# yinghansun/pympc-quadruped

Hardware: AMD Instinct MI355X
Metric: QP solves/sec (whole node), horizon=10 GRF QP, at 1/2/4/8 MI355X (higher is better)
Workload: dtype f64; 1 GPU; config2: batch 1024/GPU, horizon 10, gaits trot10, robots a1; batch_per_gpu=1024, horizon=10, global_batch=1024, parallelism=robot-sharded x1

## Files before the change

pympc-quadruped_amd/csrc/mpcqp.hip:

```cpp

#include <hip/hip_runtime.h>

#include <math.h>
#include <stdint.h>

#include <cmath>
#include <string.h>

#include <new>
#include <string>
#include <type_traits>
#include <utility>
#include <vector>

#include "mpcqp.h"

namespace {

constexpr int NX = 13;
constexpr int NU = 12;
constexpr int LANES = 64;
constexpr int kMaxN = MPCQP_MAX_HORIZON;
constexpr int kDenseN = 20;
static_assert(kMaxN >= kDenseN && 4 * kMaxN <= 2 * LANES, "stance lists cover 4 N <= 128 entries");
// ... 225 lines not shown
      "s_nop 1\n\t"
      "v_min_f32_dpp %0, %0, %0 row_bcast:31 row_mask:0xc bank_mask:0xf"
      : "+v"(v));
  return __builtin_bit_cast(float, __builtin_amdgcn_readlane(__builtin_bit_cast(int, v), 63));
}
__device__ __forceinline__ int wave_argmin_d(double v, double& vmin_out) {
  const float f = (float)v;
  const float fm = wave_min_f32(f);
  const unsigned long long cand = __ballot(f == fm);
  int l;
  if (__popcll(cand) == 1) {
    l = uni(__builtin_ctzll(cand));
    vmin_out = readlane_d(v, l);
  } else if (fm == INFINITY && __ballot(v < INFINITY) == 0ull) {
    l = 0;
    vmin_out = INFINITY;
  } else {
    const double vv = (f == fm) ? v : INFINITY;
    const double m = wave_min(vv);
    l = uni(__builtin_ctzll(__ballot(vv == m)));
    vmin_out = m;
  }
  return l;
}

__device__ __forceinline__ int wave_argmin_f32(double v, double& vmin_out) {
  const float f = (float)v;
  const float fm = wave_min_f32(f);
  const int l = uni(__builtin_ctzll(__ballot(f == fm)));
  vmin_out = readlane_d(v, l);
  return l;
}

#include "mpcqp_form.h"
#include "mpcqp_combo_asm.h"
#include "mpcqp_solve.h"
#include "mpcqp_ipm.h"
#include "mpcqp_plan.h"
#include "mpcqp_swing.h"
#include "mpcqp_kinematics.h"
#include "mpcqp_estimator.h"
#include "mpcqp_attitude.h"
static_assert(MPCQP_KIN_STRIDE == KIN_STRIDE, "geometry record: include/mpcqp.h and mpcqp_kin_leg.h agree");

__device__ __forceinline__ int xcd_robot(int bid, int B) {
  const int x = bid & 7, i = bid >> 3, q = B >> 3, r = B & 7;
  return x * q + (x < r ? x : r) + i;
}

constexpr int kOrderMax = 8192;
constexpr int kOrderSeg = 1024;
constexpr int kOrderMin = 64;
constexpr int kOrderBuckets = 256;

__device__ __forceinline__ float order_key(const float* __restrict__ x0g, const float* __restrict__ xrefg, int N,
                                           int r) {
  const float ex = x0g[(size_t)r * NX + 9] - xrefg[(size_t)r * N * NX + 9];
  const float ey = x0g[(size_t)r * NX + 10] - xrefg[(size_t)r * N * NX + 10];
  const float k = ex * ex + ey * ey;
  return k >= 0.0f && k <= 3.0e38f ? k : 0.0f;
}

__global__ __launch_bounds__(1024) void mpcqp_order_kernel(int B, int N, const float* __restrict__ x0g,
                                                           const float* __restrict__ xrefg, int* __restrict__ perm,
                                                           int mode) {
  __shared__ int hist[kOrderBuckets], cursor[kOrderBuckets];
// ... 48 lines not shown
    }
    if (lane == LANES - 1) wsum[tid >> 6] = x;
    hist[tid] = x - v;
  }
  __syncthreads();
  if (tid < kOrderBuckets) {
    int off = 0;
    for (int w = 0; w < (tid >> 6); ++w) off += wsum[w];
    hist[tid] += off;
  }
  __syncthreads();
#pragma unroll
  for (int t = 0; t < KPT; ++t) {
    const int j = tid + 1024 * t;
    if (j < len) {
      const int pos = hist[bk[t]] + atomicAdd(&cursor[bk[t]], 1);
      perm[start + stride * pos] = start + stride * j;
    }
  }
}

constexpr int kCap64 = 64;
constexpr int kIpmPerCU = 4;
template <int NM, bool FULL, bool MG>
constexpr bool ipm_within_slots() {
  return sizeof(IpmSharedT<NM, FULL, MG>) > 160 * 1024 / (kIpmPerCU + 1);
}
static_assert(ipm_within_slots<16, false, true>() && ipm_within_slots<16, true, true>() &&
                  ipm_within_slots<16, false, false>() && ipm_within_slots<16, true, false>() &&
                  ipm_within_slots<kDenseN, false, false>() && ipm_within_slots<kDenseN, true, false>() &&
                  ipm_within_slots<kMaxN, false, false>() && ipm_within_slots<kMaxN, true, false>(),
              "an interior-point layout fits more workgroups on a CU than kIpmPerCU slots");

template <bool FULL>
__global__ __launch_bounds__(Cfg<64>::NT) __attribute__((amdgpu_waves_per_eu(2, Cfg<64>::NW))) void mpcqp_kernel_64(
    KParams P, int B, const float* __restrict__ x0g, const float* __restrict__ xrefg,
    const float* __restrict__ contactg, const float* __restrict__ feetg, const float* __restrict__ robotg,
    float* __restrict__ u0g, float* __restrict__ Ug, int* __restrict__ statusg, int* __restrict__ itersg,
    int* __restrict__ queue, int* __restrict__ queue_big, int* __restrict__ queue_ipm, const int* __restrict__ perm) {
  if ((int)blockIdx.x >= B) return;
  int b = xcd_robot(blockIdx.x, B);
  if (perm) b = uni(perm[b]);
  __shared__ SharedT<64> sm;
  solve_robot<64, FULL>(P, b, sm, x0g, xrefg, contactg, feetg, robotg, u0g, Ug, statusg, itersg, queue, queue_big,
                  queue_ipm);
}

template <bool FULL>
__global__ __launch_bounds__(Cfg<96>::NT) __attribute__((amdgpu_waves_per_eu((Cfg<96>::NW + 3) / 4, (Cfg<96>::NW + 3) / 4))) void mpcqp_kernel_96(
    KParams P, const float* __restrict__ x0g, const float* __restrict__ xrefg,
    const float* __restrict__ contactg, const float* __restrict__ feetg, const float* __restrict__ robotg,
    float* __restrict__ u0g, float* __restrict__ Ug, int* __restrict__ statusg, int* __restrict__ itersg,
    int* __restrict__ queue, int* __restrict__ qout, int* __restrict__ q_ipm, int direct_B,
    const int* __restrict__ perm) {
  __shared__ SharedT<96> sm;
  const int tid = threadIdx.x;
  const int k = blockIdx.x;
  if (direct_B > 0) {
    if (k < direct_B)
      solve_robot<96, FULL>(P, perm ? uni(perm[k]) : k, sm, x0g, xrefg, contactg, feetg, robotg, u0g, Ug, statusg,
                            itersg, qout, nullptr, q_ipm);
    return;
  }
  const int cnt = uni(__hip_atomic_load(&queue[0], __ATOMIC_RELAXED, __HIP_MEMORY_SCOPE_AGENT));
  if (k < cnt) {
    const int b = uni(queue[4 + k]);
    solve_robot<96, FULL>(P, b, sm, x0g, xrefg, contactg, feetg, robotg, u0g, Ug, statusg, itersg, qout, nullptr, q_ipm);
    if (tid == 0 && atomicAdd(&queue[2], 1) == cnt - 1) {
      atomicExch(&queue[0], 0);
      atomicExch(&queue[2], 0);
    }
  }
}

template <bool FULL>
__global__ __launch_bounds__(Cfg<128>::NT) void mpcqp_kernel_128(
    KParams P, const float* __restrict__ x0g, const float* __restrict__ xrefg,
    const float* __restrict__ contactg, const float* __restrict__ feetg, const float* __restrict__ robotg,
// ... 64 lines not shown
}

struct QueueSet {
  hipStream_t stream;
  int cap;
  int* buf;
  unsigned long long used;
  hipStream_t side;
  hipEvent_t ev_fork, ev_join;
  hipEvent_t ev_done;
};

static void release_set(QueueSet& q) {
  if (q.buf) (void)hipFree(q.buf);
  if (q.ev_fork) (void)hipEventDestroy(q.ev_fork);
  if (q.ev_join) (void)hipEventDestroy(q.ev_join);
  if (q.ev_done) (void)hipEventDestroy(q.ev_done);
  q.ev_done = nullptr;
  if (q.side) (void)hipStreamDestroy(q.side);
  q.buf = nullptr;
  q.ev_fork = q.ev_join = nullptr;
  q.side = nullptr;
}

struct mpcqp_ctx {
  mpcqp_params params;
  int device;
  int stance_hint;
  int stance_min;
  int order;
  int ncu;
  std::vector<QueueSet> queues;
  unsigned long long use_clock;
  double* sscratch;
  int sslots;
  double* wdev;
  bool xr;
  double q_full[13 * 13];
  double r_full[12 * 12];
  std::vector<double*> retired;
  unsigned char* warm;
  int warm_cap;
  double dt_control;
  double gravity;
  double max_pos_error;
  double swing_height;
  double touchdown_z;
  double vel_gain;
  double kp_swing[9];
  double kd_swing[9];
  EstParams est;
  AttParams att;
  std::string err;
};

static int set_err(mpcqp_ctx* ctx, int code, const std::string& msg) {
  if (ctx) ctx->err = msg;
  return code;
}

struct DeviceScope {
  int prev = -1;
  bool ok = false;
  explicit DeviceScope(int dev) {
    if (hipGetDevice(&prev) != hipSuccess) prev = -1;
    ok = hipSetDevice(dev) == hipSuccess;
// ... 102 lines not shown
  if (hipGetDeviceCount(&ndev) != hipSuccess || device < 0 || device >= ndev) return MPCQP_ERR_HIP;
  mpcqp_ctx* ctx = new (std::nothrow) mpcqp_ctx();
  if (!ctx) return MPCQP_ERR_ALLOC;
  ctx->params = *p;
  ctx->device = device;
  ctx->stance_hint = 0;
  ctx->stance_min = 0;
  ctx->order = 1;
  ctx->ncu = 0;
  ctx->use_clock = 0;
  ctx->sscratch = nullptr;
  ctx->sslots = 0;
  ctx->wdev = nullptr;
  ctx->xr = false;
  ctx->warm = nullptr;
  ctx->warm_cap = 0;
  for (int i = 0; i < 13 * 13; ++i) ctx->q_full[i] = (i % 14 == 0) ? p->q_diag[i / 14] : 0.0;
  for (int i = 0; i < 12 * 12; ++i) ctx->r_full[i] = (i % 13 == 0) ? p->r_diag[i / 13] : 0.0;
  ctx->dt_control = 0.001;
  ctx->gravity = 9.81;
  ctx->swing_height = 0.1;
  ctx->touchdown_z = -0.0255;
  ctx->vel_gain = 0.03;
  for (int i = 0; i < 9; ++i) {
    ctx->kp_swing[i] = i % 4 == 0 ? 700.0 : 0.0;
    ctx->kd_swing[i] = i % 4 == 0 ? 20.0 : 0.0;
  }
  ctx->max_pos_error = 0.1;
  ctx->est = EstParams{0, 0.001, 9.81, 0.001, 0.0098, 0.002, 0.001, 0.1, 0.001, 100.0, 100.0, 0.0};
  ctx->att = AttParams{0.001, 9.81, 0.1, 0.0, 0.2, 0.0};
  hipDeviceProp_t prop;
  if (hipGetDeviceProperties(&prop, device) == hipSuccess) ctx->ncu = prop.multiProcessorCount;
  if (ctx->ncu <= 0) ctx->ncu = 256;
  *out = ctx;
  return MPCQP_OK;
}

int mpcqp_set_warm_start(mpcqp_ctx* ctx, void* memory, int32_t capacity) {
  if (!ctx) return MPCQP_ERR_ARG;
  if (capacity < 0 || (capacity > 0 && !memory))
    return set_err(ctx, MPCQP_ERR_ARG, "warm start: capacity < 0, or no memory for capacity > 0");
  ctx->warm = capacity > 0 ? static_cast<unsigned char*>(memory) : nullptr;
  ctx->warm_cap = capacity > 0 ? capacity : 0;
  return MPCQP_OK;
}

int mpcqp_set_order(mpcqp_ctx* ctx, int32_t mode) {
  if (!ctx) return MPCQP_ERR_ARG;
  if (mode != 0 && mode != 1) return set_err(ctx, MPCQP_ERR_ARG, "order: mode must be 0 or 1");
  ctx->order = mode;
  return MPCQP_OK;
}

int mpcqp_set_stance_hint(mpcqp_ctx* ctx, int32_t max_stance) {
  return mpcqp_set_stance_range(ctx, 0, max_stance);
}

int mpcqp_set_stance_range(mpcqp_ctx* ctx, int32_t min_stance, int32_t max_stance) {
  if (!ctx) return MPCQP_ERR_ARG;
  if (min_stance < 0 || max_stance < 0 || (max_stance > 0 && min_stance > max_stance))
    return set_err(ctx, MPCQP_ERR_ARG, "stance range: min > max or negative");
  if (min_stance > 4 * ctx->params.horizon)
    return set_err(ctx, MPCQP_ERR_ARG, "stance range: min_stance > 4 * horizon");
  ctx->stance_min = min_stance;
  ctx->stance_hint = max_stance;
  return MPCQP_OK;
// ... 71 lines not shown
                       ctx->sscratch, sbits, ctx->sslots / 32);
    ipm_done = true;
    return hipGetLastError();
  };
  auto fork_ipm = [&]() -> int {
    if (!fork || ipm_done) return MPCQP_OK;
    if (hipEventRecord(qs->ev_fork, st) != hipSuccess || hipStreamWaitEvent(qs->side, qs->ev_fork, 0) != hipSuccess)
      return set_err(ctx, MPCQP_ERR_HIP, "interior-point fork failed");
    const hipError_t le = launch_ipm(qs->side);
    if (le != hipSuccess) return set_err(ctx, MPCQP_ERR_HIP, std::string("launch (ipm): ") + hipGetErrorString(le));
    if (hipEventRecord(qs->ev_join, qs->side) != hipSuccess) return set_err(ctx, MPCQP_ERR_HIP, "join record failed");
    return MPCQP_OK;
  };
  const size_t qstride = 4 + (size_t)cap;
  int* q1 = large ? q : nullptr;
  int* perm = use_order ? q + 3 * qstride : nullptr;
  int* q2 = huge ? q + qstride : nullptr;
  int* q3 = giant ? q + 2 * qstride : nullptr;
  hipError_t e = hipSuccess;
  int fe = MPCQP_OK;
  auto failed = [&](int code) -> int {
    if (fork && ipm_done) (void)hipStreamWaitEvent(st, qs->ev_join, 0);
    if (qs) (void)hipEventRecord(qs->ev_done, st);
    return code;
  };
  if (use_order) {
    const int segs = first == 0 ? 8 : (int)((batch + kOrderSeg - 1) / kOrderSeg);
    hipLaunchKernelGGL(mpcqp_order_kernel, dim3(segs), dim3(1024), 0, st, (int)batch, kp.N, x0, xref, perm,
                       first == 0 ? 0 : 1);
    e = hipGetLastError();
    if (e != hipSuccess) return failed(set_err(ctx, MPCQP_ERR_HIP, std::string("launch (order): ") + hipGetErrorString(e)));
  }
  if (first == 0) {
    hipLaunchKernelGGL(full ? mpcqp_kernel_64<true> : mpcqp_kernel_64<false>, dim3(batch), dim3(Cfg<64>::NT),
                       kDiagLds, st, kp, (int)batch, x0, xref, contact,
                       feet, robot, u0, U, (int*)status, (int*)iters, q1, q2, q3, perm);
    e = hipGetLastError();
    if (e != hipSuccess) return failed(set_err(ctx, MPCQP_ERR_HIP, std::string("launch: ") + hipGetErrorString(e)));
    if ((fe = fork_ipm()) != MPCQP_OK) return failed(fe);
  }
  if (large && first <= 1) {
    hipLaunchKernelGGL(full ? mpcqp_kernel_96<true> : mpcqp_kernel_96<false>, dim3(batch), dim3(Cfg<96>::NT), 0, st, kp, x0, xref, contact, feet, robot,
                       u0, U, (int*)status, (int*)iters, q1, q2, q3, first == 1 ? (int)batch : 0,
                       first == 1 ? perm : nullptr);
    e = hipGetLastError();
    if (e != hipSuccess) return failed(set_err(ctx, MPCQP_ERR_HIP, std::string("launch (96): ") + hipGetErrorString(e)));
    if ((fe = fork_ipm()) != MPCQP_OK) return failed(fe);
  }
  if (huge && first <= 2) {
    hipLaunchKernelGGL(full ? mpcqp_kernel_128<true> : mpcqp_kernel_128<false>, dim3(batch), dim3(Cfg<128>::NT), 0, st, kp, x0, xref, contact, feet, robot,
                       u0, U, (int*)status, (int*)iters, q2, q3, first == 2 ? (int)batch : 0,
                       first == 2 ? perm : nullptr);
    e = hipGetLastError();
    if (e != hipSuccess) return failed(set_err(ctx, MPCQP_ERR_HIP, std::string("launch (128): ") + hipGetErrorString(e)));
    if ((fe = fork_ipm()) != MPCQP_OK) return failed(fe);
  }
  if (giant && !ipm_done) {
    e = launch_ipm(st);
    if (e != hipSuccess) return failed(set_err(ctx, MPCQP_ERR_HIP, std::string("launch (ipm): ") + hipGetErrorString(e)));
  } else if (fork && hipStreamWaitEvent(st, qs->ev_join, 0) != hipSuccess) {
    return failed(set_err(ctx, MPCQP_ERR_HIP, "interior-point join failed"));
  }
  if (qs && hipEventRecord(qs->ev_done, st) != hipSuccess) return set_err(ctx, MPCQP_ERR_HIP, "queue event record failed");
  return MPCQP_OK;
}

int mpcqp_set_weights(mpcqp_ctx* ctx, const double* Q, const double* R) {
  if (!ctx) return MPCQP_ERR_ARG;
  double q[NX * NX], r[NU * NU];
// ... 305 lines not shown
  ctx->att = AttParams{dt, gravity, kappa_ref, bias_gain, trust_window, touch_threshold};
  return MPCQP_OK;
}

int mpcqp_attitude(mpcqp_ctx* ctx, int32_t batch, int32_t flags, const float* gyro, const float* accel,
                   const int32_t* tick, int32_t iterations_between_mpc, const int32_t* gait, const float* touch,
                   double* att_state, float* quat, float* gyro_out, float* trust, int32_t* status, void* stream) {
  if (!ctx) return MPCQP_ERR_ARG;
  if (flags != 0) return set_err(ctx, MPCQP_ERR_ARG, "unknown attitude flags");
  if (batch <= 0) return set_err(ctx, MPCQP_ERR_ARG, "attitude: batch <= 0");
  if (!gyro || !accel || !att_state) return set_err(ctx, MPCQP_ERR_ARG, "null attitude input/state pointer");
  if ((uintptr_t)att_state & 15) return set_err(ctx, MPCQP_ERR_ARG, "att_state is not 16-byte aligned");
  if (gait && !tick) return set_err(ctx, MPCQP_ERR_ARG, "attitude: gait given without tick");
  if (trust && !gait && !touch)
    return set_err(ctx, MPCQP_ERR_ARG, "attitude: trust wanted with neither gait and tick nor touch");
  if (gait && iterations_between_mpc < 1) return set_err(ctx, MPCQP_ERR_ARG, "attitude: iterations_between_mpc < 1");
  static_assert(ATT_STRIDE == MPCQP_ATT_STRIDE, "record stride");
  static_assert(ATT_STATUS_OK == MPCQP_STATUS_OK && ATT_STATUS_NONFINITE == MPCQP_STATUS_NONFINITE, "status words");
  DeviceScope dev(ctx->device);
  if (!dev.ok) return set_err(ctx, MPCQP_ERR_HIP, "hipSetDevice failed");
  hipLaunchKernelGGL(mpcqp_attitude_kernel, dim3((batch + kAttThreads - 1) / kAttThreads), dim3(kAttThreads), 0,
                     (hipStream_t)stream, ctx->att, (int)batch, (int)iterations_between_mpc, gyro, accel, tick, gait,
                     touch, att_state, quat, gyro_out, trust, status);
  const hipError_t e = hipGetLastError();
  if (e != hipSuccess) return set_err(ctx, MPCQP_ERR_HIP, std::string("attitude launch: ") + hipGetErrorString(e));
  return MPCQP_OK;
}

int mpcqp_destroy(mpcqp_ctx* ctx) {
  if (ctx) {
    DeviceScope dev(ctx->device);
    for (auto& q : ctx->queues) release_set(q);
    if (ctx->sscratch) (void)hipFree(ctx->sscratch);
    if (ctx->wdev) (void)hipFree(ctx->wdev);
    for (double* o : ctx->retired) (void)hipFree(o);
  }
  delete ctx;
  return MPCQP_OK;
}

const char* mpcqp_last_error(const mpcqp_ctx* ctx) { return ctx ? ctx->err.c_str() : "null context"; }

}
```

pympc-quadruped_amd/csrc/mpcqp_form.h:

```cpp

template <int NM>
struct alignas(16) FormT {
  static constexpr int IN_XREF = IN_CONTACT + 4 * NM, IN_END = IN_XREF + NX * NM;
  float in[IN_END];
  double K[3][NU];
  double G[3][NU];
  double E0[NM][16];
  double E1[NM][8];
  double ii[9];
  double rz[2];
  double minv;
  double q[16];
  double qf[NX * NX];
  double es[2][NM][NX];
  double X[2][NX][NU];
  double QX[2][NX][NU];
};
using Form = FormT<kDenseN>;

struct alignas(16) FormY {
  d2 Y[NU * NU];
  double rd2[NU];
  double Yf[3][NU * NU];
  double rf2[NU * NU];
// ... 180 lines not shown
    double a = 0.0;
#pragma unroll
    for (int j = 0; j < NX; ++j) a = fma(f.qf[i * NX + j], f.X[w][j][c], a);
    f.QX[w][i][c] = a;
  }
  for (int e = tid; e < N * NX; e += NT) {
    const int t = e / NX, sc = e % NX;
    double a0 = 0.0, a1 = 0.0;
#pragma unroll
    for (int j = 0; j < NX; ++j) {
      a0 = fma(f.qf[sc * NX + j], f.es[0][t][j], a0);
      a1 = fma(f.qf[sc * NX + j], f.es[1][t][j], a1);
    }
    f.E0[t][sc] = a0;
    if (sc < 6) f.E1[t][sc] = a1;
  }
  fsync<NT>();
  for (int e = tid; e < 3 * NU * NU; e += NT) {
    const int w = e / (NU * NU), c1 = (e / NU) % NU, c2 = e % NU;
    const int xa = w == 2 ? 1 : 0, qb = w == 0 ? 0 : 1;
    double a = 0.0;
#pragma unroll
    for (int i = 0; i < NX; ++i) a = fma(f.X[xa][i][c1], f.QX[qb][i][c2], a);
    fy.Yf[w][c1 * NU + c2] = a;
  }
}

template <class F>
__device__ __forceinline__ void form_weights(const KParams& P, F& f, FormY& fy, int tid) {
  if (tid < NX) f.q[tid] = P.q[tid];
  if (tid < NU) fy.rd2[tid] = 2.0 * P.r[tid];
}

template <int NT, bool SPLIT = false, class F, class MT>
__device__ __forceinline__ void form_model(const KParams& P, F& f, FormY& fy, MT& mt, int N, int tid) {
  static_assert(!SPLIT || NT == 2 * LANES, "the split setup is laid out for two waves");
  constexpr int CS = SPLIT ? LANES : NT;
  constexpr int T_SUF = SPLIT ? LANES : 64 - 16;
  constexpr int T_CONE = SPLIT ? 2 * LANES - 18 : 64 - 18;
  const float* const rbs = f.in + IN_ROBOT;
  const double h = P.dt;
  double qsuf = 0.0;
  if constexpr (SPLIT)
    if (tid >= T_SUF && tid < T_SUF + NX) qsuf = P.q[tid - T_SUF];
  const double yaw = (double)f.in[IN_X0 + 2];
  double sy, cy;
  sincos(yaw, &sy, &cy);
  const double c = f32r(cy), s = f32r(sy);
  auto rz = [&](int a, int bb) -> double {
    return a == 2 ? (bb == 2 ? 1.0 : 0.0) : (bb == 2 ? 0.0 : (a == bb ? c : (a == 0 ? -s : s)));
  };
  if (!SPLIT || tid < LANES) {
    const int i = tid / 3, j = tid % 3;
    auto ib = [&](int a, int bb) -> double {
      const int lo = a < bb ? a : bb, hi = a < bb ? bb : a;
      const int idx = lo == 0 ? hi : (lo == 1 ? 2 + hi : 5);
      return (double)rbs[1 + idx];
    };
    if (tid < 9) f.ii[tid] = f32r(rz(i, 0) * ib(0, j) + rz(i, 1) * ib(1, j) + rz(i, 2) * ib(2, j));
    form_weights(P, f, fy, tid);
    if (tid == 0) {
      f.rz[0] = c;
      f.rz[1] = s;
      f.minv = f32r(1.0 / (double)rbs[0]);
    }
    fsync<CS>();
    double iw = 0.0;
    if (tid < 9) iw = f32r(f.ii[3 * i] * rz(j, 0) + f.ii[3 * i + 1] * rz(j, 1) + f.ii[3 * i + 2] * rz(j, 2));
// ... 22 lines not shown
#pragma unroll
      for (int a = 0; a < 3; ++a) kk[a] = f32r(f.ii[3 * a] * sk0 + f.ii[3 * a + 1] * sk1 + f.ii[3 * a + 2] * sk2);
      f.K[i][col] = kk[i];
      f.G[i][col] = rz(0, i) * kk[0] + rz(1, i) * kk[1] + rz(2, i) * kk[2];
    }
  }
  if (tid >= T_CONE && tid < T_CONE + 18) {
    const int k18 = tid - T_CONE;
    double nx = rbs[9], ny = rbs[10], nz = rbs[11];
    const double nn = sqrt(nx * nx + ny * ny + nz * nz);
    if (!(nn > 0.0)) {
      nx = 0.0; ny = 0.0; nz = 1.0;
    } else {
      nx /= nn; ny /= nn; nz /= nn;
    }
    double t1x = 1.0 - nx * nx, t1y = -nx * ny, t1z = -nx * nz;
    const double tn = sqrt(t1x * t1x + t1y * t1y + t1z * t1z);
    t1x /= tn; t1y /= tn; t1z /= tn;
    const double t2x = ny * t1z - nz * t1y, t2y = nz * t1x - nx * t1z, t2z = nx * t1y - ny * t1x;
    const double mu = rbs[7];
    const int rr = k18 / 3, k = k18 % 3;
    const double nk = k == 0 ? nx : (k == 1 ? ny : nz);
    const double t1k = k == 0 ? t1x : (k == 1 ? t1y : t1z);
    const double t2k = k == 0 ? t2x : (k == 1 ? t2y : t2z);
    const double val = rr == 0 ? t1k + mu * nk
                     : rr == 1 ? -t1k + mu * nk
                     : rr == 2 ? t2k + mu * nk
                     : rr == 3 ? -t2k + mu * nk
                     : rr == 4 ? nk : -nk;
    mt.rows[rr][k] = val;
    if (k18 == 0) mt.fz0_implied = mu > 0.0;
  }
  if (P.wfull) {
    form_model_full<NT>(P, f, fy, N, tid);
    return;
  }
  if (tid >= T_SUF && tid < T_SUF + NX) {
    const int sc = tid - T_SUF;
    const float* xin = f.in + IN_X0;
    const double q = SPLIT ? qsuf : f.q[sc];
    double x0s = (double)xin[sc], n1 = 0.0, n2 = 0.0;
    const double g12 = (double)xin[12];
    if (sc < 3) n1 = h * (rz(0, sc) * (double)xin[6] + rz(1, sc) * (double)xin[7] + rz(2, sc) * (double)xin[8]);
    else if (sc < 6) n1 = h * (double)xin[6 + sc] + (sc == 5 ? 0.5 * h * h * g12 : 0.0);
    else if (sc == 11) n1 = h * g12;
    if (sc == 5) n2 = h * h * g12;
    double e0 = 0.0, e1 = 0.0;
    for (int t = N - 1; t >= 0; --t) {
      const double k = (double)(t + 1);
      const double e = x0s + k * n1 + 0.5 * k * (k - 1.0) * n2 - (double)f.in[F::IN_XREF + t * NX + sc];
      e0 = fma(q, e, e0);
      e1 = fma((double)t * q, e, e1);
      f.E0[t][sc] = e0;
      if (sc < 6) f.E1[t][sc] = e1;
    }
  }
  fsync<NT>();
  {
    const double minv2 = f.minv * f.minv;
    const double ca = 0.25 * h * h * h * h, cb = h * h;
    for (int k = tid; k < NU * NU; k += NT) {
      const int c1 = k / NU, c2 = k % NU;
      double ya = 0.0, yb = 0.0;
#pragma unroll
      for (int i = 0; i < 3; ++i) {
        ya = fma(f.G[i][c1] * f.q[i], f.G[i][c2], ya);
        yb = fma(f.K[i][c1] * f.q[6 + i], f.K[i][c2], yb);
      }
      if (c1 % 3 == c2 % 3) {
        ya = fma(f.q[3 + c1 % 3], minv2, ya);
        yb = fma(f.q[9 + c1 % 3], minv2, yb);
      }
      fy.Y[k] = d2{ca * ya, cb * yb};
    }
  }
}

template <class F, class MT>
__device__ __forceinline__ double form_g(const KParams& P, const F& f, const MT& mt, int a) {
  const double h = P.dt;
  const int sf = a / 3, ax = a % 3;
  const int j = mt.foot_t[sf], cc = 3 * mt.foot_leg[sf] + ax;
  const double* E0 = f.E0[j];
  const double* E1 = f.E1[j];
  const double al0 = f.G[0][cc] * E0[0] + f.G[1][cc] * E0[1] + f.G[2][cc] * E0[2] + E0[3 + ax] * f.minv;
  const double al1 = f.G[0][cc] * E1[0] + f.G[1][cc] * E1[1] + f.G[2][cc] * E1[2] + E1[3 + ax] * f.minv;
  const double be0 = f.K[0][cc] * E0[6] + f.K[1][cc] * E0[7] + f.K[2][cc] * E0[8] + E0[9 + ax] * f.minv;
  return 2.0 * (0.5 * h * h * ((double)(1 - 2 * j) * al0 + 2.0 * al1) + h * be0);
}
// ... 28 lines not shown
```

pympc-quadruped_amd/csrc/mpcqp_solve.h:

```cpp

template <int NV>
struct Cfg {
  static constexpr int TW = NV == 96 ? 6 : 8;
  static constexpr int NW = NV * NV / (4 * TW * LANES);
  static constexpr int NT = NW * LANES;
  static constexpr int TCN = NV / TW;
  static constexpr int RPW = 256 / TCN;
  static constexpr int CPL = NV / 32;
  static constexpr int VPL = (NV + LANES - 1) / LANES;
  static constexpr int VEC = VPL * LANES;
  static constexpr int TS = TW == 8 ? 10 : TW;
  static constexpr int SVEC = TW == 8 ? TCN * TS : VEC;
  static_assert(NW * LANES * 4 * TW == NV * NV, "4 x TW tiles");
  static_assert(TCN == 8 || TCN == 16, "tile rows are reduced over 8 or 16 lanes");
};

template <int NV>
struct FormArea {
  Form f;
  FormY fy;
  d2 mt_tab[kDenseN * kDenseN];
};
template <int NV>
struct alignas(16) SharedT {
  static constexpr bool kPair = NV <= 96;
  union {
    FormArea<NV> fa;
    double ht[NV * NV];
  };
  RobotMeta mt;
  union {
    struct {
      alignas(16) double zc[2][Cfg<NV>::VEC];
      alignas(16) double vz[2][Cfg<NV>::VEC];
    };
    double wb[4 * Cfg<NV>::VEC];
    alignas(16) double swz[(NV >= 96 ? 4 : 2) * Cfg<NV>::SVEC];
  };
  alignas(16) double vr[2][Cfg<NV>::VEC];
  union {
    struct {
      alignas(16) double vx[Cfg<NV>::VEC];
      alignas(16) double gv[Cfg<NV>::VEC];
    };
    alignas(16) double vr2[2][Cfg<NV>::VEC];
  };
  alignas(16) double rl[Cfg<NV>::VEC];
  alignas(16) double zp[NV == 128 ? 2 * Cfg<NV>::SVEC : 2];
  alignas(16) double tv[Cfg<NV>::VEC];
  alignas(16) double yv[Cfg<NV>::VEC];
  double wmax[Cfg<NV>::NW];
  int choice;
};
static_assert(sizeof(FormArea<64>) <= sizeof(double) * 64 * 64, "formulation scratch exceeds the H copy");
static_assert(sizeof(SharedT<64>) <= 160 * 1024 / 4, "class 64 holds four robots per CU");

constexpr int DPP_SHL1 = 0x101;
constexpr int DPP_ROR8 = 0x128;

__device__ __forceinline__ double dpp_shl1(double v) {
  const long long bits = __double_as_longlong(v);
  const int lo = __builtin_amdgcn_update_dpp(0, (int)bits, DPP_SHL1, 0xF, 0xF, true);
  const int hi = __builtin_amdgcn_update_dpp(0, (int)(bits >> 32), DPP_SHL1, 0xF, 0xF, true);
  return __longlong_as_double(((long long)hi << 32) | (unsigned int)lo);
}
template <int TCN>
__device__ __forceinline__ double tile_reduce(const double (&acc)[4], int lane) {
  const bool hi4 = (lane & 4) != 0;
  double k2[2];
#pragma unroll
  for (int k = 0; k < 2; ++k) {
    const double send = hi4 ? acc[k] : acc[2 + k];
    const double keep = hi4 ? acc[2 + k] : acc[k];
    k2[k] = keep + dpp_d<DPP_HMIRROR>(send);
  }
  const bool hi2 = (lane & 2) != 0;
  const double send = hi2 ? k2[0] : k2[1];
  const double keep = hi2 ? k2[1] : k2[0];
  double y = keep + dpp_d<DPP_XOR2>(send);
  y += dpp_d<DPP_XOR1>(y);
  if constexpr (TCN == 16) y += dpp_d<DPP_ROR8>(y);
  return y;
}
template <int TCN>
__device__ __forceinline__ int trow(int tr, int lane) {
// ... 18 lines not shown
      b2 = fma(M[r][c + 1], vs[c + 1], b2);
    }
    acc[r] = a + b2;
  }
  return tile_reduce<TCN>(acc, lane);
}

template <int C0, int TW>
__device__ __forceinline__ void colcombo_u(const double (&Pm)[4][TW], const double (&Rm)[4][TW], double a0, double a1,
                                           double a2, bool rlive, double (&zq)[4], double (&rq)[4]) {
#pragma unroll
  for (int r = 0; r < 4; ++r) zq[r] = fma(a2, Pm[r][C0 + 2], fma(a1, Pm[r][C0 + 1], a0 * Pm[r][C0]));
  if (rlive) {
#pragma unroll
    for (int r = 0; r < 4; ++r) rq[r] = fma(a2, Rm[r][C0 + 2], fma(a1, Rm[r][C0 + 1], a0 * Rm[r][C0]));
  } else {
#pragma unroll
    for (int r = 0; r < 4; ++r) rq[r] = 0.0;
  }
}

template <int NT>
__device__ __forceinline__ void write_empty_t(int b, int tid, int N, int code, float* u0g, float* Ug, int* statusg,
                                              int* itersg) {
  if (tid < 12) u0g[(size_t)b * 12 + tid] = 0.f;
  if (Ug)
    for (int k = tid; k < N * 12; k += NT) Ug[(size_t)b * N * 12 + k] = 0.f;
  if (tid == 0) {
    if (statusg) statusg[b] = code;
    if (itersg) itersg[b] = 0;
  }
}

template <int NV, bool FULL>
__device__ __forceinline__ void solve_robot(const KParams& P, int b, SharedT<NV>& sm, const float* __restrict__ x0g,
                                            const float* __restrict__ xrefg, const float* __restrict__ contactg,
                                            const float* __restrict__ feetg, const float* __restrict__ robotg,
                                            float* __restrict__ u0g, float* __restrict__ Ug, int* __restrict__ statusg,
                                            int* __restrict__ itersg, int* __restrict__ queue,
                                            int* __restrict__ queue_big = nullptr,
                                            int* __restrict__ queue_ipm = nullptr) {
  using C = Cfg<NV>;
  constexpr int NT = C::NT, TCN = C::TCN, CPL = C::CPL, VPL = C::VPL, RPW = C::RPW, TW = C::TW;
  const int tid = threadIdx.x;
  const int lane = tid & (LANES - 1), wave = uni(tid >> 6);
  const int tr = tid / TCN, tc = tid % TCN;
  const int N = P.N;
#ifdef MPCQP_STAMPS
  unsigned long long stamps_[7];
  unsigned long long substamps_[3] = {0, 0, 0};
  unsigned long long secacc_ = 0, seclast_ = 0;
  int seccur_ = 7;
#endif
  STAMP(0);
#ifdef MPCQP_STAMPS
  const unsigned long long rt0_ = __builtin_amdgcn_s_memrealtime();
#endif

  Form& smf = sm.fa.f;
  FormY& smfy = sm.fa.fy;
  constexpr bool kSplitSetup = NV == 64;
  auto fill_mt_tab = [&] {
    if constexpr (!FULL) {
      for (int e = tid; e < N * N; e += NT) {
        const int ja = e / N, jb = e - ja * N;
        const int mx = ja > jb ? ja : jb;
        const int d = ja > jb ? ja - jb : jb - ja;
        const int m = N - mx;
        const int ta = (m * (4 * m * m - 1)) / 3 + 2 * d * m * m;
        sm.fa.mt_tab[e] = d2{(double)ta, (double)m};
      }
    }
  };
  bool staged;
  if constexpr (kSplitSetup) {
    staged = form_stage<NT>(smf, N, b, tid, x0g, xrefg, contactg, feetg, robotg, fill_mt_tab);
  } else {
    staged = form_stage<NT>(smf, N, b, tid, x0g, xrefg, contactg, feetg, robotg);
  }
  if (!staged) {
    write_empty_t<NT>(b, tid, N, MPCQP_STATUS_NONFINITE, u0g, Ug, statusg, itersg);
    return;
  }
  SUBSTAMP(0);
  int S;
  if constexpr (kSplitSetup) {
    S = form_stance(smf, sm.mt, N, lane, wave == 0);
  } else {
    if (wave == 0) form_stance(smf, sm.mt, N, lane);
    fsync<NT>();
    S = uni(sm.mt.S);
  }
  const int n = 3 * S, m = 6 * S;
  if (n > NV) {
    int* qn = queue;
    if (queue_big && n > 96) qn = queue_big;
    if (queue_ipm && n > 128) qn = queue_ipm;
    if (qn) {
      if (tid == 0) qn[4 + atomicAdd(&qn[0], 1)] = b;
      return;
    }
    write_empty_t<NT>(b, tid, N, MPCQP_STATUS_TOO_LARGE, u0g, Ug, statusg, itersg);
    return;
  }

  SUBSTAMP(1);
  form_model<NT, kSplitSetup>(P, smf, smfy, sm.mt, N, tid);
  SUBSTAMP(2);
  if constexpr (kSplitSetup) {
    if (tid >= NT - NV) {
      const int a = tid - (NT - NV);
      sm.gv[a] = a < n ? form_g(P, smf, sm.mt, a) : 0.0;
    }
    fsync<NT>();
  } else {
    fill_mt_tab();
    fsync<NT>();
    if (tid < NV) sm.gv[tid] = tid < n ? form_g(P, smf, sm.mt, tid) : 0.0;
  }
  STAMP(1);

  auto hcols = [&](int (&cj)[TW], int (&cc)[TW]) {
#pragma unroll
    for (int c = 0; c < TW; ++c) {
      const int col = TW * tc + c;
      const int sb = col < n ? col / 3 : 0;
      cj[c] = sm.mt.foot_t[sb];
      cc[c] = 3 * sm.mt.foot_leg[sb] + col % 3;
    }
  };
  auto hrow = [&](int r, const int (&cj)[TW], const int (&cc)[TW], double (&h)[TW]) {
    const int row = 4 * tr + r;
    const int sa = row < n ? row / 3 : 0;
    const int ja = sm.mt.foot_t[sa];
    const int car = 3 * sm.mt.foot_leg[sa] + row % 3;
    const double r2 = smfy.rd2[row < n ? car : 0];
#pragma unroll
    for (int c = 0; c < TW; ++c) {
      const int col = TW * tc + c;
      double hv;
      if constexpr (FULL) hv = form_h_full(smfy, N, ja, car, cj[c], cc[c]);
      else hv = form_h_tab(smfy, sm.fa.mt_tab[ja * N + cj[c]], car, cc[c]) + (row == col ? r2 : 0.0);
      h[c] = (row < n && col < n) ? hv : (row == col ? 1.0 : 0.0);
    }
  };
  double W[4][TW];
  {
    int cj[TW], cc[TW];
    hcols(cj, cc);
#pragma unroll
    for (int r = 0; r < 4; ++r) hrow(r, cj, cc, W[r]);
  }
  fsync<NT>();
// ... 137 lines not shown
  for (int r = 0; r < 4; ++r)
#pragma unroll
    for (int c = 0; c < TW; ++c) W[r][c] = -W[r][c];
  if constexpr (TW == 8) {
    if (tc == (tr >> 1)) {
      const double odd = (double)(tr & 1);
#pragma unroll
      for (int r = 0; r < 4; ++r) {
        const double dv = fma(odd, W[r][4 + r], (1.0 - odd) * W[r][r]);
        if (4 * tr + r < n) wd = fmax(wd, dv);
      }
    }
  } else {
#pragma unroll
    for (int r = 0; r < 4; ++r)
#pragma unroll
      for (int c = 0; c < TW; ++c)
        if (4 * tr + r == TW * tc + c && 4 * tr + r < n) wd = fmax(wd, W[r][c]);
  }
  wd = wave_max_d(wd);
  if (lane == 0) sm.wmax[wave] = wd;
  fsync<NT>();
#pragma unroll
  for (int r = 0; r < 4; ++r) {
    const int row = 4 * tr + r;
    const int sf = row / 3;
    const int c0 = row < n ? 3 * sf - TW * tc : NV;
    const int wi = 9 * sf + 3 * (row - 3 * sf) - c0;
#pragma unroll
    for (int c = 0; c < TW; ++c)
      if ((unsigned)(c - c0) < 3u) sm.wb[wi + c] = W[r][c];
  }
  STAMP(3);

  {
    const double y = tile_matvec4<TCN, TW>(W, sm.gv, tc, lane);
    if (twriter<TCN>(lane)) sm.vx[trow<TCN>(tr, lane)] = -y;
  }
  fsync<NT>();
  double wscale = sm.wmax[0];
#pragma unroll
  for (int w = 1; w < C::NW; ++w) wscale = fmax(wscale, sm.wmax[w]);
  wscale = sgpr_d(wscale);
  const float qfloor = fmaxf((float)(1e-9 * wscale), 1e-30f);

  int cz[CPL], crt[CPL];
  double s[CPL];
  constexpr bool kCurKey = NV <= 96;
  float qm[CPL];
  auto cdot = [&](const double* v, int k) -> double {
    const double* a = sm.mt.rows[crt[k]];
    const double* vf = v + cz[k];
    return a[0] * vf[0] + a[1] * vf[1] + a[2] * vf[2];
  };
  auto cbound = [&](int k) -> double {
    return crt[k] == 5 ? sm.mt.ub[cz[k] / 3] : 0.0;
  };
#pragma unroll
  for (int k = 0; k < CPL; ++k) {
    const int c = lane + LANES * k;
    const bool ok = c < m;
    cz[k] = ok ? 3 * (c / 6) : 0;
    crt[k] = ok ? c % 6 : 0;
    const bool live = ok && !(crt[k] == 4 && sm.mt.fz0_implied);
    s[k] = live ? cdot(sm.vx, k) + cbound(k) : INFINITY;
    const double* a = sm.mt.rows[crt[k]];
// ... 538 lines not shown
  STAMP(4);

  fsync<NT>();
  if (wave == 0) {
#pragma unroll
    for (int k = 0; k < VPL; ++k) sm.vx[lane + LANES * k] = x[k];
  }
  fsync<NT>();
  {
    int bad = 0;
#pragma unroll
    for (int k = 0; k < CPL; ++k) {
      if (lane + LANES * k < m) {
        const double v = cdot(sm.vx, k) + cbound(k);
        bad |= (v < -1e-6) || !isfinite(v);
      }
    }
#pragma unroll
    for (int k = 0; k < VPL; ++k)
      if ((occ[k] >> lane) & 1ull) bad |= (u[k] < -1e-9);
    if (__any(bad) && status == MPCQP_STATUS_OK) status = MPCQP_STATUS_MAX_ITER;
  }
  STAMP(5);
  STAMP(6);

#ifdef MPCQP_STAMPS
  if (Ug) {
    unsigned long long* dst = (unsigned long long*)Ug + (size_t)b * kStampU64;
    if (tid == 0) {
      for (int i = 0; i < 7; ++i) dst[i] = stamps_[i];
      dst[7] = rt0_;
      dst[8] = __builtin_amdgcn_s_memrealtime();
      for (int i = 0; i < 3; ++i) dst[9 + i] = substamps_[i];
    }
    if (lane < 24) dst[32 + 24 * wave + lane] = secacc_;
    if (lane == 0)
      dst[16 + wave] = (unsigned)__builtin_amdgcn_s_getreg((31 << 11) | 4) |
                       ((unsigned long long)(__builtin_amdgcn_s_getreg((3 << 11) | 20) & 15) << 32) |
                       ((unsigned long long)blockIdx.x << 40);
  }
  Ug = nullptr;
#endif
  if (wave == 0) {
    if (lane < 12) {
      const int sidx = sm.mt.stance_of[lane / 3];
      u0g[(size_t)b * 12 + lane] = sidx >= 0 ? (float)sm.vx[3 * sidx + lane % 3] : 0.f;
    }
    if (Ug) {
      for (int k = lane; k < N * 12; k += LANES) {
        const int sidx = sm.mt.stance_of[k / 3];
        Ug[(size_t)b * N * 12 + k] = sidx >= 0 ? (float)sm.vx[3 * sidx + k % 3] : 0.f;
      }
    }
    if (lane == 0) {
      if (statusg) statusg[b] = status;
      if (itersg) itersg[b] = it;
    }
  }
}
```

Measured before the change: 10.52 million QP/s.

## Raise wave priority during setup for the hardest robot per CU

Adds a device-side priority table indexed by XCC and CU id. During setup, each class-64 workgroup posts its ordering key there with an atomic max, then reads the slot back before the formation barrier. The workgroup holding the largest key on its CU raises its wave priority with s_setprio through the Hessian/factor stage, so that the slowest solve on each CU finishes sooner and the kernel tail shrinks. The cost is an extra key computation, global atomics, an epoch counter with a periodic table reset, and some risk of starving co-resident workgroups.

```diff
diff --git a/pympc-quadruped_amd/csrc/mpcqp.hip b/pympc-quadruped_amd/csrc/mpcqp.hip
--- a/pympc-quadruped_amd/csrc/mpcqp.hip
+++ b/pympc-quadruped_amd/csrc/mpcqp.hip
@@ -281,6 +281,7 @@
   return l;
 }
 
+constexpr int kPrioTab = 4096;
 #include "mpcqp_form.h"
 #include "mpcqp_combo_asm.h"
 #include "mpcqp_solve.h"
@@ -395,18 +396,22 @@
                   ipm_within_slots<kMaxN, false, false>() && ipm_within_slots<kMaxN, true, false>(),
               "an interior-point layout fits more workgroups on a CU than kIpmPerCU slots");
 
-template <bool FULL>
+template <bool FULL, bool PRIO = false>
 __global__ __launch_bounds__(Cfg<64>::NT) __attribute__((amdgpu_waves_per_eu(2, Cfg<64>::NW))) void mpcqp_kernel_64(
     KParams P, int B, const float* __restrict__ x0g, const float* __restrict__ xrefg,
     const float* __restrict__ contactg, const float* __restrict__ feetg, const float* __restrict__ robotg,
     float* __restrict__ u0g, float* __restrict__ Ug, int* __restrict__ statusg, int* __restrict__ itersg,
-    int* __restrict__ queue, int* __restrict__ queue_big, int* __restrict__ queue_ipm, const int* __restrict__ perm) {
+    int* __restrict__ queue, int* __restrict__ queue_big, int* __restrict__ queue_ipm, const int* __restrict__ perm,
+    unsigned long long* __restrict__ prio_tab, unsigned prio_epoch) {
   if ((int)blockIdx.x >= B) return;
   int b = xcd_robot(blockIdx.x, B);
   if (perm) b = uni(perm[b]);
+  unsigned long long prio_val = 0ull;
+  if constexpr (PRIO)
+    prio_val = ((unsigned long long)prio_epoch << 32) | __float_as_uint(order_key(x0g, xrefg, P.N, b));
   __shared__ SharedT<64> sm;
-  solve_robot<64, FULL>(P, b, sm, x0g, xrefg, contactg, feetg, robotg, u0g, Ug, statusg, itersg, queue, queue_big,
-                  queue_ipm);
+  solve_robot<64, FULL, PRIO>(P, b, sm, x0g, xrefg, contactg, feetg, robotg, u0g, Ug, statusg, itersg, queue, queue_big,
+                  queue_ipm, prio_tab, prio_val);
 }
 
 template <bool FULL>
@@ -537,6 +542,8 @@
   int ncu;
   std::vector<QueueSet> queues;
   unsigned long long use_clock;
+  unsigned long long* prio_tab;
+  unsigned prio_epoch;
   double* sscratch;
   int sslots;
   double* wdev;
@@ -705,6 +712,21 @@
   hipDeviceProp_t prop;
   if (hipGetDeviceProperties(&prop, device) == hipSuccess) ctx->ncu = prop.multiProcessorCount;
   if (ctx->ncu <= 0) ctx->ncu = 256;
+  ctx->prio_tab = nullptr;
+  ctx->prio_epoch = 0;
+  {
+    DeviceScope dev(device);
+    if (!dev.ok || hipMalloc(&ctx->prio_tab, sizeof(unsigned long long) * kPrioTab) != hipSuccess) {
+      delete ctx;
+      return MPCQP_ERR_ALLOC;
+    }
+    if (hipMemsetAsync(ctx->prio_tab, 0, sizeof(unsigned long long) * kPrioTab, nullptr) != hipSuccess ||
+        hipStreamSynchronize(nullptr) != hipSuccess) {
+      (void)hipFree(ctx->prio_tab);
+      delete ctx;
+      return MPCQP_ERR_HIP;
+    }
+  }
   *out = ctx;
   return MPCQP_OK;
 }
@@ -842,9 +864,17 @@
     if (e != hipSuccess) return failed(set_err(ctx, MPCQP_ERR_HIP, std::string("launch (order): ") + hipGetErrorString(e)));
   }
   if (first == 0) {
-    hipLaunchKernelGGL(full ? mpcqp_kernel_64<true> : mpcqp_kernel_64<false>, dim3(batch), dim3(Cfg<64>::NT),
-                       kDiagLds, st, kp, (int)batch, x0, xref, contact,
-                       feet, robot, u0, U, (int*)status, (int*)iters, q1, q2, q3, perm);
+    const bool prio = batch <= resident;
+    if (prio && ++ctx->prio_epoch == 0) {
+      if (hipMemsetAsync(ctx->prio_tab, 0, sizeof(unsigned long long) * kPrioTab, st) != hipSuccess)
+        return failed(set_err(ctx, MPCQP_ERR_HIP, "priority table reset failed"));
+      ctx->prio_epoch = 1;
+    }
+    hipLaunchKernelGGL(prio ? (full ? mpcqp_kernel_64<true, true> : mpcqp_kernel_64<false, true>)
+                            : (full ? mpcqp_kernel_64<true> : mpcqp_kernel_64<false>),
+                       dim3(batch), dim3(Cfg<64>::NT), kDiagLds, st, kp, (int)batch, x0, xref, contact,
+                       feet, robot, u0, U, (int*)status, (int*)iters, q1, q2, q3, perm,
+                       prio ? ctx->prio_tab : (unsigned long long*)nullptr, ctx->prio_epoch);
     e = hipGetLastError();
     if (e != hipSuccess) return failed(set_err(ctx, MPCQP_ERR_HIP, std::string("launch: ") + hipGetErrorString(e)));
     if ((fe = fork_ipm()) != MPCQP_OK) return failed(fe);
@@ -1216,6 +1246,7 @@
     DeviceScope dev(ctx->device);
     for (auto& q : ctx->queues) release_set(q);
     if (ctx->sscratch) (void)hipFree(ctx->sscratch);
+    if (ctx->prio_tab) (void)hipFree(ctx->prio_tab);
     if (ctx->wdev) (void)hipFree(ctx->wdev);
     for (double* o : ctx->retired) (void)hipFree(o);
   }
diff --git a/pympc-quadruped_amd/csrc/mpcqp_form.h b/pympc-quadruped_amd/csrc/mpcqp_form.h
--- a/pympc-quadruped_amd/csrc/mpcqp_form.h
+++ b/pympc-quadruped_amd/csrc/mpcqp_form.h
@@ -236,8 +236,12 @@
   if (tid < NU) fy.rd2[tid] = 2.0 * P.r[tid];
 }
 
-template <int NT, bool SPLIT = false, class F, class MT>
-__device__ __forceinline__ void form_model(const KParams& P, F& f, FormY& fy, MT& mt, int N, int tid) {
+struct FormNoHook {
+  __device__ __forceinline__ void operator()() const {}
+};
+template <int NT, bool SPLIT = false, class F, class MT, class PB = FormNoHook>
+__device__ __forceinline__ void form_model(const KParams& P, F& f, FormY& fy, MT& mt, int N, int tid,
+                                           PB pre_barrier = PB()) {
   static_assert(!SPLIT || NT == 2 * LANES, "the split setup is laid out for two waves");
   constexpr int CS = SPLIT ? LANES : NT;
   constexpr int T_SUF = SPLIT ? LANES : 64 - 16;
@@ -326,6 +330,7 @@
     if (k18 == 0) mt.fz0_implied = mu > 0.0;
   }
   if (P.wfull) {
+    pre_barrier();
     form_model_full<NT>(P, f, fy, N, tid);
     return;
   }
@@ -349,6 +354,7 @@
       if (sc < 6) f.E1[t][sc] = e1;
     }
   }
+  pre_barrier();
   fsync<NT>();
   {
     const double minv2 = f.minv * f.minv;
diff --git a/pympc-quadruped_amd/csrc/mpcqp_solve.h b/pympc-quadruped_amd/csrc/mpcqp_solve.h
--- a/pympc-quadruped_amd/csrc/mpcqp_solve.h
+++ b/pympc-quadruped_amd/csrc/mpcqp_solve.h
@@ -51,6 +51,7 @@
   alignas(16) double yv[Cfg<NV>::VEC];
   double wmax[Cfg<NV>::NW];
   int choice;
+  int prio;
 };
 static_assert(sizeof(FormArea<64>) <= sizeof(double) * 64 * 64, "formulation scratch exceeds the H copy");
 static_assert(sizeof(SharedT<64>) <= 160 * 1024 / 4, "class 64 holds four robots per CU");
@@ -135,14 +136,16 @@
   }
 }
 
-template <int NV, bool FULL>
+template <int NV, bool FULL, bool PRIO = false>
 __device__ __forceinline__ void solve_robot(const KParams& P, int b, SharedT<NV>& sm, const float* __restrict__ x0g,
                                             const float* __restrict__ xrefg, const float* __restrict__ contactg,
                                             const float* __restrict__ feetg, const float* __restrict__ robotg,
                                             float* __restrict__ u0g, float* __restrict__ Ug, int* __restrict__ statusg,
                                             int* __restrict__ itersg, int* __restrict__ queue,
                                             int* __restrict__ queue_big = nullptr,
-                                            int* __restrict__ queue_ipm = nullptr) {
+                                            int* __restrict__ queue_ipm = nullptr,
+                                            unsigned long long* __restrict__ prio_tab = nullptr,
+                                            unsigned long long prio_val = 0ull) {
   using C = Cfg<NV>;
   constexpr int NT = C::NT, TCN = C::TCN, CPL = C::CPL, VPL = C::VPL, RPW = C::RPW, TW = C::TW;
   const int tid = threadIdx.x;
@@ -186,6 +189,16 @@
     return;
   }
   SUBSTAMP(0);
+  unsigned long long* prio_slot = nullptr;
+  static_assert(!PRIO || NV == 64, "the setup priority is class 64's");
+  if constexpr (PRIO) {
+    if (prio_tab && wave == 1) {
+      const unsigned hw = (unsigned)__builtin_amdgcn_s_getreg((31 << 11) | 4);
+      const unsigned xcc = (unsigned)__builtin_amdgcn_s_getreg((3 << 11) | 20);
+      prio_slot = prio_tab + ((((xcc & 15u) << 8) | ((hw >> 8) & 0xffu)) & (unsigned)(kPrioTab - 1));
+      if (lane == 0) (void)__hip_atomic_fetch_max(prio_slot, prio_val, __ATOMIC_RELAXED, __HIP_MEMORY_SCOPE_AGENT);
+    }
+  }
   int S;
   if constexpr (kSplitSetup) {
     S = form_stance(smf, sm.mt, N, lane, wave == 0);
@@ -208,13 +221,23 @@
   }
 
   SUBSTAMP(1);
-  form_model<NT, kSplitSetup>(P, smf, smfy, sm.mt, N, tid);
+  unsigned long long prio_seen = ~0ull;
+  if constexpr (PRIO) {
+    form_model<NT, kSplitSetup>(P, smf, smfy, sm.mt, N, tid, [&] {
+      if (prio_slot) prio_seen = __hip_atomic_load(prio_slot, __ATOMIC_RELAXED, __HIP_MEMORY_SCOPE_AGENT);
+    });
+  } else {
+    form_model<NT, kSplitSetup>(P, smf, smfy, sm.mt, N, tid);
+  }
   SUBSTAMP(2);
   if constexpr (kSplitSetup) {
     if (tid >= NT - NV) {
       const int a = tid - (NT - NV);
       sm.gv[a] = a < n ? form_g(P, smf, sm.mt, a) : 0.0;
     }
+    if constexpr (PRIO) {
+      if (prio_slot && lane == 0) sm.prio = prio_seen == prio_val;
+    }
     fsync<NT>();
   } else {
     fill_mt_tab();
@@ -222,6 +245,11 @@
     if (tid < NV) sm.gv[tid] = tid < n ? form_g(P, smf, sm.mt, tid) : 0.0;
   }
   STAMP(1);
+  bool prio_raised = false;
+  if constexpr (PRIO) {
+    prio_raised = prio_tab && uni(sm.prio) != 0;
+    if (prio_raised) __builtin_amdgcn_s_setprio(3);
+  }
 
   auto hcols = [&](int (&cj)[TW], int (&cc)[TW]) {
 #pragma unroll
@@ -425,6 +453,9 @@
       if ((unsigned)(c - c0) < 3u) sm.wb[wi + c] = W[r][c];
   }
   STAMP(3);
+  if constexpr (PRIO) {
+    if (prio_raised) __builtin_amdgcn_s_setprio(0);
+  }
 
   {
     const double y = tile_matvec4<TCN, TW>(W, sm.gv, tc, lane);
@@ -1029,6 +1060,7 @@
       dst[7] = rt0_;
       dst[8] = __builtin_amdgcn_s_memrealtime();
       for (int i = 0; i < 3; ++i) dst[9 + i] = substamps_[i];
+      dst[12] = prio_raised ? 1ull : 0ull;
     }
     if (lane < 24) dst[32 + 24 * wave + lane] = secacc_;
     if (lane == 0)
```

After: 10.91 million QP/s (median of 6 runs). 3.7% higher.
